# ViV99/slam-experiments

Measured on NVIDIA B200. Metric: hamming_pairs_per_sec, higher is better.
Workload: dtype u8

## Files before the change

### slam_experiments_b200/csrc/hm_tc.cu

```cuda
#include <math.h>
#include <stdlib.h>

#include <mutex>
#include <type_traits>

#include <cuda_fp16.h>

#include "hm_common.cuh"
#include "hm_tcgen05.cuh"

#ifndef HM_F4_TILE_N
#define HM_F4_TILE_N 128
#endif

namespace hm {

namespace {

constexpr int kRowBlock = 128;
constexpr int kMBlocks = 2;
constexpr int kBlockM = kRowBlock * kMBlocks;
constexpr int kSlabBytes = kRowBlock * 128;
constexpr int kPadRows = HM_PREPARED_TILE_ROWS;
constexpr int kTmemCols = 512;
// ... 59 lines not shown
    {
        const __half2 h = *reinterpret_cast<const __half2*>(&p);
        return hi ? __high2float(h) : __low2float(h);
    }
    static constexpr uint32_t kLowestBits = 0xFF800000u;
};

template <class C> __host__ __device__ constexpr int row_block_bytes() { return kRowBlock * C::kRowBytes; }
template <class C> __host__ __device__ constexpr int a_bytes() { return kMBlocks * row_block_bytes<C>(); }
template <class C> __host__ __device__ constexpr int b_stage_bytes() { return C::kTileN * C::kRowBytes; }
template <class C> __host__ __device__ constexpr int epilogue_warps() { return 4 * kMBlocks * C::kColSplit; }
template <class C> __host__ __device__ constexpr int control_warps() { return C::kRegisterHandover ? 4 : 2; }
template <class C> __host__ __device__ constexpr int threads() { return 32 * (control_warps<C>() + epilogue_warps<C>()); }
constexpr int kHandoverBytes = kBlockM * 16;
constexpr int kBarrierBytes = 512;
template <class C> __host__ __device__ constexpr int smem_bytes() { return 1024 + a_bytes<C>() + C::kStages * b_stage_bytes<C>() + kBarrierBytes + kHandoverBytes; }
static_assert((2 * CoreF4::kStages + 1 + 2 * CoreF4::kUnits) * 8 + 16 <= kBarrierBytes, "barrier block");
static_assert((2 * CoreI8::kStages + 1 + 2 * CoreI8::kUnits) * 8 + 16 <= kBarrierBytes, "barrier block");
__host__ __device__ constexpr int ct_gcd(int a, int b) { return b == 0 ? a : ct_gcd(b, a % b); }
template <class C> __host__ __device__ constexpr int issuer_period() { return C::kStages / ct_gcd(C::kStages, C::kUnits) * C::kUnits; }
constexpr int kScaleCols = 32;
constexpr int kScaleCol = kTmemCols - kScaleCols;
static_assert(CoreF4::kUnits * CoreF4::kTileN <= kScaleCol, "accumulator units must end before the scale factors");

struct PrepareParams {
    const uint8_t* bits;
    long long n, stride, batch_stride;
    long long padded_rows;
    uint8_t* out;
};

// ... 246 lines not shown
#define HM_SCAN_FLAT64 1
#endif
#ifndef HM_FLOOR_DENSE_TILES
#define HM_FLOOR_DENSE_TILES 32
#endif
#ifndef HM_FLOOR_LATE_MASK
#define HM_FLOOR_LATE_MASK 15
#endif

#ifndef HM_F4_A_TMEM
#define HM_F4_A_TMEM 0
#endif
constexpr int kATmemCol = 384;
constexpr int kATmemColsPerBlock = 32;

template <class C>
__device__ __forceinline__ void issue_half(int h, uint32_t a_block, uint32_t b_stage, uint32_t tmem_d, uint32_t idesc,
                                           uint32_t tmem_sf)
{
    constexpr int kHalf = C::kSlabs * 2;
#pragma unroll
    for (int jj = 0; jj < kHalf; ++jj) {
        const int j = h * kHalf + jj;
        const int slab = j >> 2, k = j & 3;
        const uint64_t db = ptx::kmajor_sw128_desc_from_lo(b_stage + ((slab * kSlabBytes + k * 32) >> 4));
        if constexpr (C::kScales && HM_F4_A_TMEM) {
            ptx::mma_mxf4_ts(tmem_d, a_block + 8 * j, db, idesc, tmem_sf, tmem_sf + kScaleCols / 2, j != 0);
        } else {
            const uint64_t da = ptx::kmajor_sw128_desc_from_lo(a_block + ((slab * kSlabBytes + k * 32) >> 4));
            if constexpr (C::kScales) ptx::mma_mxf4_ss(tmem_d, da, db, idesc, tmem_sf, tmem_sf + kScaleCols / 2, j != 0);
            else                      ptx::mma_i8_ss(tmem_d, da, db, idesc, j != 0);
        }
    }
}

template <class C, int kMode>
__device__ __forceinline__ void tc_knn2_body(const TcParams& P)
{
    constexpr bool kFloor = kMode == 1;
    using Acc = typename C::Acc;
    constexpr int kStages = C::kStages;
    constexpr int kUnits = C::kUnits;
    constexpr int kABytes = a_bytes<C>();
    constexpr int kBStageBytes = b_stage_bytes<C>();
    constexpr int kRowBlockBytes = row_block_bytes<C>();
    constexpr int kTileN = C::kTileN;

    extern __shared__ uint8_t smem_raw[];
    uint8_t* smem = smem_raw + ((1024u - (ptx::smem_u32(smem_raw) & 1023u)) & 1023u);
    uint8_t* smem_a = smem;
    uint8_t* smem_b = smem + kABytes;
    uint64_t* bars = reinterpret_cast<uint64_t*>(smem + kABytes + kStages * kBStageBytes);
    uint64_t* full_bar = bars;
    uint64_t* empty_bar = bars + kStages;
    uint64_t* a_full_bar = bars + 2 * kStages;
    uint64_t* tmem_full_bar = bars + 2 * kStages + 1;
    uint64_t* tmem_empty_bar = tmem_full_bar + kUnits;
    uint32_t* tmem_base_slot = reinterpret_cast<uint32_t*>(tmem_empty_bar + kUnits);
    uint32_t* smem_base_slot = tmem_base_slot + 2;
    ulonglong2* handover = reinterpret_cast<ulonglong2*>(smem + kABytes + kStages * kBStageBytes + kBarrierBytes);

    const int warp = __shfl_sync(0xffffffffu, threadIdx.x >> 5, 0);
    const int lane = threadIdx.x & 31;
    if (threadIdx.x == 0) cta_mark(P, 0);
    if (threadIdx.x == 0 && (blockIdx.x | blockIdx.y | blockIdx.z) == 0 && P.clock_probe) {
        unsigned long long t;
        asm volatile("mov.u64 %0, %%globaltimer;" : "=l"(t));
        P.clock_probe[0] = (long long)t;
        P.clock_probe[1] = clock64();
    }
    const int qb = blockIdx.x;
    const int split = blockIdx.y;
    const int b = blockIdx.z;

    const uint32_t cs = ptx::cluster_nctarank();
    const uint32_t crank = ptx::cluster_ctarank();
    const uint16_t cmask = (uint16_t)((1u << cs) - 1);
    const bool has_a = qb < P.q_blocks_valid;
    auto rows_present = [&]() -> long long { return P.nq_dyn ? min((long long)__ldg(P.nq_dyn + b), P.nq) : P.nq; };
    if (P.nq_dyn && (long long)(qb - (int)crank) * kBlockM >= rows_present()) return;

    const int tile_begin = split * P.tiles_per_split;
    const int tile_end = min(tile_begin + P.tiles_per_split, P.ntiles);
    const int my_tiles = tile_end - tile_begin;

    constexpr int kProducerWarp = kIssuerLast ? epilogue_warps<C>() : 0;
    constexpr int kIssuerWarp = kIssuerLast ? epilogue_warps<C>() + 1 : 1;
    constexpr int kFirstEpiWarp = kIssuerLast ? 0 : 2;
    static_assert(kIssuerLast || !C::kRegisterHandover, "the control warps must form the last warpgroup");
    static_assert(!C::kRegisterHandover || (epilogue_warps<C>() == 16 && threads<C>() == 640),
                  "the register budget (4 x 32 + 16 x 112 = 20 x 96) assumes 20 warps launched at 96 registers");
    if (warp == kProducerWarp && lane == 0) {
        *smem_base_slot = ptx::smem_u32(smem);
        for (int i = 0; i < kStages; ++i) {
            ptx::mbar_init(&full_bar[i], 1);
            ptx::mbar_init(&empty_bar[i], cs);
        }
        ptx::mbar_init(a_full_bar, 1);
        for (int i = 0; i < kUnits; ++i) {
            ptx::mbar_init(&tmem_full_bar[i], 1);
            ptx::mbar_init(&tmem_empty_bar[i], 4 * C::kColSplit);
        }
        ptx::fence_barrier_init();
        ptx::fence_proxy_async();
    } else if (warp == kIssuerWarp) {
        ptx::tmem_alloc(tmem_base_slot, kTmemCols);
        ptx::tmem_relinquish();
    }
    ptx::tc_fence_before();
    if (cs > 1) ptx::cluster_sync();
    else __syncthreads();
    ptx::tc_fence_after();
    const uint32_t tmem_base = *tmem_base_slot;

    if constexpr (C::kScales) {
        if (warp >= kFirstEpiWarp && warp < kFirstEpiWarp + 4) {
            uint32_t ones[32];
#pragma unroll
            for (int i = 0; i < 32; ++i) ones[i] = 0x7F7F7F7Fu;
            const uint32_t taddr = tmem_base + ((uint32_t)((warp & 3) * 32) << 16) + kScaleCol;
            static_assert(kScaleCols == 32, "one x32 store per lane quarter");
            ptx::tmem_st_32x32(taddr, ones);
// ... 42 lines not shown
                const int blk = o >> 10, rem = o & 1023;
                const int rr = (rem >> 3) & 7;
                const int r = ((rem >> 6) << 3) | rr;
                const int c = (rem & 7) ^ rr;
                const long long qrow = (long long)qb * kBlockM + blk * kRowBlock + r;
                uint4 v = make_uint4(0, 0, 0, 0);
                if (qrow < nq_eff) {
                    const long long srow = qidx ? (long long)__ldg(qidx + qrow) : qrow;
                    v = expand_bits_e2m1(*reinterpret_cast<const unsigned*>(qsrc + srow * P.q_bits_stride + c * 4));
                }
                reinterpret_cast<uint4*>(smem_a)[o] = v;
            }
            ptx::fence_proxy_async();
        }
        ptx::tc_fence_before();
        __syncthreads();
        ptx::tc_fence_after();
    }

    if (threadIdx.x == 0) cta_mark(P, 1);
    ulonglong2 my_keys = make_ulonglong2(kNoMatch, kNoMatch);
    long long my_row = -1;
    int my_row_in_cta = 0;

    auto run_producer = [&]() {
        if (lane == 0) {
            if (has_a && !P.qbits && !(C::kScales && HM_F4_A_TMEM)) {
                const uint8_t* qsrc = P.qprep + ((long long)b * P.q_padded + (long long)qb * kBlockM) * C::kRowBytes;
                ptx::mbar_arrive_expect_tx(a_full_bar, kABytes);
                ptx::bulk_g2s(smem_a, qsrc, kABytes, a_full_bar);
            }
            const uint8_t* tsrc = P.tprep + (long long)b * P.t_padded * C::kRowBytes;
            const uint32_t piece = kBStageBytes / cs;
            for (int i = 0; i < (HM_TC_EXPERIMENT >= 5 ? 0 : my_tiles); ++i) {
                const int stage = i % kStages;
                const uint32_t use = i / kStages;
#if HM_TC_EXPERIMENT < 4
                bounded_wait(&empty_bar[stage], (use & 1) ^ 1, P.error_flag);
#endif
                trace_mark(P, i, 0);
                ptx::mbar_arrive_expect_tx(&full_bar[stage], kBStageBytes);
                uint8_t* dst = smem_b + stage * kBStageBytes + crank * piece;
                const uint8_t* src = tsrc + (long long)(tile_begin + i) * kBStageBytes + crank * piece;
                if (cs > 1) ptx::bulk_g2s_multicast(dst, src, piece, &full_bar[stage], cmask);
                else        ptx::bulk_g2s(dst, src, piece, &full_bar[stage]);
            }
        }
    };
    auto run_issuer = [&]() {
        const bool leader = ptx::elect_one();
        const uint32_t idesc = C::kScales ? ptx::make_mxf4_idesc(kRowBlock, kTileN) : ptx::make_i8_idesc(kRowBlock, kTileN);
        constexpr bool kATmem = C::kScales && HM_F4_A_TMEM;
        const uint32_t a_addr = kATmem ? tmem_base + kATmemCol : ptx::smem_u32(smem_a) >> 4;
        constexpr uint32_t kABlockStep = kATmem ? (uint32_t)kATmemColsPerBlock : (uint32_t)(kRowBlockBytes >> 4);
        const uint32_t b_addr = ptx::smem_u32(smem_b) >> 4;
        const uint32_t tmem_sf = tmem_base + kScaleCol;
        if (has_a && !P.qbits && !(C::kScales && HM_F4_A_TMEM)) bounded_wait(a_full_bar, 0, P.error_flag);
        constexpr int kPeriod = issuer_period<C>();
        static_assert(kPeriod % kStages == 0 && (2 * kPeriod) % kUnits == 0 && ((2 * kPeriod / kUnits) & 1) == 0,
                      "unit parities must repeat with the period");
        uint32_t sphase = 0;
        bool ready0 = false;
        for (int base = 0; base < my_tiles; base += kPeriod) {
#pragma unroll
            for (int j = 0; j < kPeriod; ++j) {
                if (base + j < my_tiles) {
                    const int stage = j % kStages;
                    const uint32_t full_par = sphase ^ ((j / kStages) & 1);
                    const int unit_a = (2 * j) % kUnits, unit_b = (2 * j + 1) % kUnits;
                    const uint32_t par_a = (((2 * j) / kUnits) & 1) ^ 1, par_b = (((2 * j + 1) / kUnits) & 1) ^ 1;
                    const uint32_t b_stage = b_addr + stage * (kBStageBytes >> 4);
                    if (leader) trace_mark(P, base + j, 7);
                    if (!ready0) {
#if HM_TC_EXPERIMENT < 4
                        bounded_wait(&full_bar[stage], full_par, P.error_flag);
#endif
#if HM_TC_EXPERIMENT < 3
                        bounded_wait(&tmem_empty_bar[unit_a], par_a, P.error_flag);
#endif
                    }
                    if (leader) trace_mark(P, base + j, 1);
                    ptx::tc_fence_after();
                    if (leader) issue_half<C>(0, a_addr, b_stage, tmem_base + unit_a * kTileN, idesc, tmem_sf);
#if HM_TC_EXPERIMENT >= 3
                    const bool ready1 = true;
#else
                    const bool ready1 = __all_sync(0xffffffffu, ptx::mbar_test_wait(&tmem_empty_bar[unit_b], par_b));
#endif
                    if (leader) {
                        issue_half<C>(1, a_addr, b_stage, tmem_base + unit_a * kTileN, idesc, tmem_sf);
#if HM_TC_EXPERIMENT != 6 && HM_COMMIT_MODE == 0
                        ptx::tc_commit(&tmem_full_bar[unit_a]);
#endif
                    }
                    if (!ready1) bounded_wait(&tmem_empty_bar[unit_b], par_b, P.error_flag);
                    if (leader) trace_mark(P, base + j, 6);
                    ptx::tc_fence_after();
                    if (leader) issue_half<C>(0, a_addr + kABlockStep, b_stage, tmem_base + unit_b * kTileN, idesc, tmem_sf);
                    ready0 = false;
                    if (base + j + 1 < my_tiles) {
                        const int n = j + 1;
#if HM_TC_EXPERIMENT >= 4
                        ready0 = true;
#else
                        ready0 = __all_sync(0xffffffffu,
                                            ptx::mbar_test_wait(&full_bar[n % kStages], sphase ^ ((n / kStages) & 1))
#if HM_TC_EXPERIMENT < 3
                                            && ptx::mbar_test_wait(&tmem_empty_bar[(2 * n) % kUnits], (((2 * n) / kUnits) & 1) ^ 1)
#endif
                                            );
#endif
                    }
                    if (leader) {
                        issue_half<C>(1, a_addr + kABlockStep, b_stage, tmem_base + unit_b * kTileN, idesc, tmem_sf);
#if HM_TC_EXPERIMENT == 6 || HM_COMMIT_MODE == 1
                        ptx::tc_commit(&tmem_full_bar[unit_a]);
#endif
                        ptx::tc_commit(&tmem_full_bar[unit_b]);
                        if (cs > 1) ptx::tc_commit_multicast(&empty_bar[stage], cmask);
                        else        ptx::tc_commit(&empty_bar[stage]);
                    }
                }
            }
            sphase ^= (kPeriod / kStages) & 1;
        }
        __syncwarp();
    };
    auto run_epilogue = [&]() {
        constexpr int kCols = kTileN / C::kColSplit;
        const int quarter = warp & 3;
        const int mblk = ((warp - kFirstEpiWarp) >> 2) & 1;
        const int half = (warp - kFirstEpiWarp) >> 3;
        const int row_in_cta = mblk * kRowBlock + quarter * 32 + lane;
        const long long row = (long long)qb * kBlockM + row_in_cta;
        Top2<Acc> s;
        s.v1 = s.v2 = C::lowest();
        s.i1 = s.i2 = 0;
#pragma unroll
        for (int e = 0; e < 4; ++e) s.sa[e] = s.sb[e] = 0;
        s.f = C::floor_from(0);
#if HM_TC_TRACE
        s.slow = 0;
#endif
        unsigned floor_code = 0;
        const long long first_row = (long long)tile_begin * kTileN;
        const unsigned limit = (unsigned)min((long long)my_tiles * kTileN, P.nt - first_row);
        const uint32_t bars_addr = ptx::lds_volatile_u32(ptx::smem_u32(smem_base_slot)) + kABytes + kStages * kBStageBytes;
        const uint32_t unit_full_addr = bars_addr + (2 * kStages + 1) * 8;
        const uint32_t unit_empty_addr = unit_full_addr + kUnits * 8;
        int unit = mblk;
        uint32_t unit_use = 0;
        unsigned floor_pending = 0;
        auto refresh_floor = [&](int i) {
            if constexpr (kFloor) {
                if (i < HM_FLOOR_DENSE_TILES || (i & HM_FLOOR_LATE_MASK) == 0) {
                    floor_code = max(floor_code, floor_pending);
                    s.f = C::max2(s.f, C::floor_from(floor_code));
                    if (row < P.nq) {
                        unsigned* floor_ptr = P.row_floor + ((long long)b * P.nq + row);
                        const unsigned e = C::valid(s.v2) ? C::encode(s.v2) : 0u;
                        if (e > floor_code) { atomicMax(floor_ptr, e); floor_code = e; }
                        floor_pending = __ldcg(floor_ptr);
                    }
                }
// ... 28 lines not shown
                }
                scan_chunk<C, kMode>(r0, colbase, s);
                scan_chunk<C, kMode>(r1, colbase + 32, s);
                scan_chunk<C, kMode>(r2, colbase + 64, s);
                scan_chunk<C, kMode>(r3, colbase + 96, s);
            } else {
                if constexpr (kCols == 64) {
                    uint32_t r[64];
#if HM_TC_EXPERIMENT < 2
                    ptx::tmem_ld_32x64(taddr, r);
                    refresh_floor(i);
                    tmem_ld_fence64(r);
#endif
                    ptx::tc_fence_before();
                    __syncwarp();
                    if (HM_ARRIVE_ELECT ? ptx::elect_one() : lane == 0) ptx::mbar_arrive_addr(unit_empty_addr + unit * 8);
#if HM_TC_EXPERIMENT != 0
                    unit += 2;
                    if (unit >= kUnits) { unit -= kUnits; ++unit_use; }
                    return;
#endif
                    mask_tail<C, 64>(r, colbase, limit);
#if HM_SCAN_FLAT64
                    scan_chunk<C, kMode, 8>(r, colbase, s);
#else
                    scan_chunk<C, kMode>(r, colbase, s);
                    scan_chunk<C, kMode>(r + 32, colbase + 32, s);
#endif
                } else if constexpr (kCols == 32) {
                    uint32_t r[32];
                    ptx::tmem_ld_32x32(taddr, r);
// ... 49 lines not shown
        if (kMode != 2) fold_group(s.v2, s.i2, s.sb);
        else my_keys.y = kNoMatch;
        if (half == 1) handover[row_in_cta] = my_keys;
        else my_row = row;
        my_row_in_cta = row_in_cta;
    };

    auto run_tail = [&](auto worker_tag) {
        constexpr bool kWorker = decltype(worker_tag)::value;
        ptx::tc_fence_before();
        if (cs > 1) ptx::cluster_sync();
        else __syncthreads();
        if (kWorker && threadIdx.x == 0) cta_mark(P, 3);
        if (warp == kIssuerWarp) {
            ptx::tc_fence_after();
            ptx::tmem_dealloc(tmem_base, kTmemCols);
        }
        if (kWorker && my_row >= 0 && my_row < rows_present()) {
            if constexpr (C::kColSplit == 2) {
                const ulonglong2 o = handover[my_row_in_cta];
                top2_insert(my_keys.x, my_keys.y, o.x);
                top2_insert(my_keys.x, my_keys.y, o.y);
            }
            unsigned long long* out = P.out + (long long)split * P.out_split_stride + ((long long)b * P.nq + my_row) * 2;
            *reinterpret_cast<ulonglong2*>(out) = my_keys;
            if (!P.counters) select_candidate(P.sel, b, my_keys);
        }
        if (P.counters) {
            int* flag = reinterpret_cast<int*>(tmem_base_slot + 1);
            if (last_cta_arrives(&P.counters[(long long)b * gridDim.x + qb], (unsigned)P.splits, flag)) {
                const long long row = (long long)qb * kBlockM + threadIdx.x;
// ... 8 lines not shown
            }
        }
        if (kWorker && threadIdx.x == 0) cta_mark(P, 4);
        if (kWorker && threadIdx.x == 0 && (blockIdx.x | blockIdx.y | blockIdx.z) == 0 && P.clock_probe) {
            unsigned long long t;
            asm volatile("mov.u64 %0, %%globaltimer;" : "=l"(t));
            P.clock_probe[2] = (long long)t;
            P.clock_probe[3] = clock64();
        }
    };

    if constexpr (C::kRegisterHandover) {
        if (warp >= kProducerWarp) {
            asm volatile("setmaxnreg.dec.sync.aligned.u32 32;\n");
            if (warp == kProducerWarp) run_producer();
            else if (warp == kIssuerWarp) run_issuer();
            run_tail(std::false_type{});
            return;
        }
        asm volatile("setmaxnreg.inc.sync.aligned.u32 112;\n");
        run_epilogue();
        run_tail(std::true_type{});
    } else {
        if (warp == kProducerWarp) run_producer();
        else if (warp == kIssuerWarp) run_issuer();
        else run_epilogue();
        run_tail(std::true_type{});
    }
}

__global__ void __launch_bounds__(threads<CoreI8>(), 1) hm_i8_knn2_kernel(const TcParams P) { tc_knn2_body<CoreI8, 0>(P); }
__global__ void __launch_bounds__(threads<CoreF4>(), 1) hm_f4_knn2_kernel(const TcParams P) { tc_knn2_body<CoreF4, 0>(P); }
__global__ void __launch_bounds__(threads<CoreI8>(), 1) hm_i8_knn2_floor_kernel(const TcParams P) { tc_knn2_body<CoreI8, 1>(P); }
__global__ void __launch_bounds__(threads<CoreF4>(), 1) hm_f4_knn2_floor_kernel(const TcParams P) { tc_knn2_body<CoreF4, 1>(P); }
__global__ void __launch_bounds__(threads<CoreI8>(), 1) hm_i8_knn1_kernel(const TcParams P) { tc_knn2_body<CoreI8, 2>(P); }
__global__ void __launch_bounds__(threads<CoreF4>(), 1) hm_f4_knn1_kernel(const TcParams P) { tc_knn2_body<CoreF4, 2>(P); }

using KernelFn = void (*)(const TcParams);
template <class C> KernelFn kernel_of(int mode = 0);
template <> KernelFn kernel_of<CoreI8>(int mode) { return mode == 1 ? hm_i8_knn2_floor_kernel : mode == 2 ? hm_i8_knn1_kernel : hm_i8_knn2_kernel; }
template <> KernelFn kernel_of<CoreF4>(int mode) { return mode == 1 ? hm_f4_knn2_floor_kernel : mode == 2 ? hm_f4_knn1_kernel : hm_f4_knn2_kernel; }

struct TcPlan {
    int ntiles, splits, tiles_per_split;
    int cluster;
    long long qblocks;
};

int floor_max_tiles()
{
    static int v = -1;
    if (v < 0) {
        const char* e = getenv("HM_FLOOR_MAX_TILES");
        v = e ? atoi(e) : 0x7fffffff;
    }
    return v;
}

int floor_min_tiles_unsplit()
{
    static int v = -1;
    if (v < 0) {
        const char* e = getenv("HM_FLOOR_MIN_TILES_UNSPLIT");
// ... 18 lines not shown

int current_device_slot()
{
    int dev = 0;
    if (cudaGetDevice(&dev) != cudaSuccess) { cudaGetLastError(); dev = 0; }
    return (dev >= 0 && dev < kMaxDevices) ? dev : -1;
}

template <class C>
cudaError_t ensure_smem_opt_in()
{
    static bool done[kMaxDevices] = {};
    const int dev = current_device_slot();
    std::lock_guard<std::mutex> lock(g_launch_state_mu);
    if (dev >= 0 && done[dev]) return cudaSuccess;
    for (int mode = 0; mode < 3; ++mode) {
        const cudaError_t e = cudaFuncSetAttribute(kernel_of<C>(mode), cudaFuncAttributeMaxDynamicSharedMemorySize, smem_bytes<C>());
        if (e != cudaSuccess) return e;
    }
    if (dev >= 0) done[dev] = true;
    return cudaSuccess;
}

template <class C>
int resident_ctas(int cs, int sm_count)
{
    static int cache[kMaxDevices][5] = {};
    if (cs <= 1) return sm_count;
    const int dev = current_device_slot();
    if (dev >= 0) {
        std::lock_guard<std::mutex> lock(g_launch_state_mu);
        if (cache[dev][cs]) return cache[dev][cs];
    }
    int v = sm_count;
// ... 21 lines not shown
    }
    return v;
}

template <class C>
int prologue_tiles()
{
    static int v = -1;
    if (v < 0) {
        const char* e = getenv("HM_PROLOGUE_TILES");
        v = e ? atoi(e) : C::kPrologueTiles;
    }
    return v;
}

int cluster_min_tiles()
{
    static int v = -1;
    if (v < 0) {
        const char* e = getenv("HM_CLUSTER_MIN_TILES");
        v = e ? atoi(e) : 1024;
    }
    return v;
}

template <class C>
TcPlan plan_tc_cluster(long long nq, long long nt, int batch, int sm_count, int cluster)
{
    TcPlan pl{};
    const long long qb = ceil_div(nq, kBlockM);
// ... 41 lines not shown
    const TcPlan pl = plan_tc<C>(nq, nt, batch, sm_count);
    return (size_t)pl.splits * batch * nq * 2 * sizeof(unsigned long long);
}

inline size_t zeroed_bytes(long long row_blocks, long long rows) { return counters_bytes(row_blocks) + counters_bytes((rows + 1) / 2 * 2); }

template <class C>
size_t workspace_bytes_of(long long nq, long long nt, int batch, int sm_count, bool with_prepare)
{
    size_t b = 256 + zeroed_bytes(plan_tc<C>(nq, nt, batch, sm_count).qblocks * batch, nq * batch) + partials_bytes<C>(nq, nt, batch, sm_count);
    b = (b + 1023) & ~(size_t)1023;
    if (with_prepare) b += (size_t)(padded_rows<C>(nq) + padded_rows<C>(nt)) * C::kRowBytes * batch;
    return b;
}

template <class C>
int launch_prepared(const void* qprep, long long nq, const void* tprep, long long nt, int batch,
                    unsigned long long train_base, unsigned long long* out, void* ws, size_t ws_bytes,
                    int sm_count, cudaStream_t stream, const unsigned long long** out_partials,
                    int* out_groups, const ExchangeArgs* exchange, bool top1 = false, const QueryBits* qbits = nullptr,
                    const SelectArgs* select = nullptr)
{
    HM_CUDA_CHECK(ensure_smem_opt_in<C>());
    const TcPlan pl = plan_tc<C>(nq, nt, batch, sm_count);
    if ((long long)pl.ntiles * C::kTileN > (1ll << 32)) {
        set_error("train set too large for 32-bit trainIdx");
        return HM_ERR_UNSUPPORTED;
    }
    const bool keep_partials = out == nullptr;
    const size_t cbytes = zeroed_bytes(pl.qblocks * batch, nq * batch);
// ... 44 lines not shown
        P.out = partials;
        P.out_split_stride = rows * 2;
    }
    const bool fused_exchange = exchange && exchange->world > 1;
    if (fused_exchange) {
        if (batch != 1 || keep_partials) {
            set_error("fused exchange needs batch == 1 and an output buffer");
            return HM_ERR_INVALID_ARGUMENT;
        }
        static_assert(kBlockM == kExchangeRows, "flag granularity = query block");
        P.xch = *exchange;
        P.out = partials;
        P.out_split_stride = rows * 2;
    }
    bool zero_block = false;
    const bool floor_eligible = !top1 && !P.nq_dyn && pl.tiles_per_split <= floor_max_tiles() &&
                                (pl.splits > 1 || (C::kColSplit > 1 && pl.ntiles >= floor_min_tiles_unsplit()));
    if (floor_eligible) {
        P.row_floor = reinterpret_cast<unsigned*>(reinterpret_cast<uint8_t*>(counters) + counters_bytes(pl.qblocks * batch));
        zero_block = true;
    }
    if ((pl.splits > 1 || fused_exchange) && !keep_partials) {
        P.counters = counters;
        P.final_out = out;
        zero_block = true;
    } else if (!(pl.splits > 1 || keep_partials)) {
        P.out = out;
        P.out_split_stride = 0;
    }
    static const bool keep_floors = getenv("HM_KEEP_FLOORS") != nullptr;
    if (zero_block) HM_CUDA_CHECK(cudaMemsetAsync(counters, 0, keep_floors ? counters_bytes(pl.qblocks * batch) : cbytes, stream));
    if (pl.qblocks > 0x7FFFFFFFll || pl.splits > 65535 || batch > 65535) {
        set_error("grid too large");
        return HM_ERR_UNSUPPORTED;
    }
    cudaLaunchConfig_t cfg{};
    cfg.gridDim = dim3((unsigned)pl.qblocks, (unsigned)pl.splits, (unsigned)batch);
    cfg.blockDim = dim3(threads<C>());
    cfg.dynamicSmemBytes = smem_bytes<C>();
    cfg.stream = stream;
    cudaLaunchAttribute attr[1];
    attr[0].id = cudaLaunchAttributeClusterDimension;
    attr[0].val.clusterDim.x = (unsigned)pl.cluster;
    attr[0].val.clusterDim.y = 1;
    attr[0].val.clusterDim.z = 1;
    cfg.attrs = attr;
    cfg.numAttrs = 1;
    profile_mark(true, stream);
    cudaError_t le = cudaLaunchKernelEx(&cfg, kernel_of<C>(P.row_floor ? 1 : top1 ? 2 : 0), P);
    profile_mark(false, stream);
    if (le != cudaSuccess) {
        set_error("cudaLaunchKernelEx(tensor-core k-NN kernel, cluster %d) failed: %s", pl.cluster, cudaGetErrorString(le));
        return HM_ERR_CUDA;
    }
    HM_CUDA_CHECK(cudaGetLastError());
    if (trace_path) {
        static long long host[kTraceTiles * kTraceSlots];
        HM_CUDA_CHECK(cudaStreamSynchronize(stream));
        HM_CUDA_CHECK(cudaMemcpy(host, P.trace, sizeof(host), cudaMemcpyDeviceToHost));
        {
            const size_t nctas = (size_t)pl.qblocks * pl.splits * batch;
            long long* rec = (long long*)malloc(nctas * kCtaSlots * sizeof(long long));
            if (rec && cudaMemcpy(rec, P.trace + kTraceTiles * kTraceSlots, nctas * kCtaSlots * sizeof(long long), cudaMemcpyDeviceToHost) == cudaSuccess) {
                char path[1024];
// ... 153 lines not shown
    const size_t head = workspace_bytes_of<C>(p.nq, p.nt, p.batch, sm_count, false);
    uint8_t* tprep = static_cast<uint8_t*>(ws) + head + (size_t)padded_rows<C>(p.nq) * C::kRowBytes * p.batch;
    int rc = launch_prepare_of<C>(p.t, p.nt, p.t_stride, p.t_batch_stride, p.batch, tprep, stream);
    if (rc != HM_OK) return rc;
    QueryBits qb{};
    qb.bits = p.q; qb.stride = p.q_stride; qb.batch_stride = p.q_batch_stride;
    qb.index = list; qb.index_batch_stride = p.nq; qb.nq_dyn = count;
    return launch_prepared<C>(nullptr, p.nq, tprep, p.nt, p.batch, 0, out, ws, head, sm_count, stream, nullptr, nullptr,
                              nullptr, true, &qb);
}

template <class C>
static void describe_of(long long nq, long long nt, int batch, int sm_count, bool top1, char* buf, size_t n)
{
    const TcPlan pl = plan_tc<C>(nq, nt, batch, sm_count);
    const bool floor = !top1 && pl.splits > 1 && pl.tiles_per_split <= floor_max_tiles();
    snprintf(buf, n, "hm_%s_knn%s%s_kernel grid=(%lld,%d,%d) cluster=%d tiles_per_cta=%d", C::kScales ? "f4" : "i8",
             top1 ? "1" : "2", floor ? "_floor" : "", pl.qblocks, pl.splits, batch, pl.cluster, pl.tiles_per_split);
}

void describe_tc_launch(long long nq, long long nt, int batch, int sm_count, int variant, bool top1, char* buf, size_t n)
{
    if (variant == HM_VARIANT_F4) describe_of<CoreF4>(nq, nt, batch, sm_count, top1, buf, n);
    else                          describe_of<CoreI8>(nq, nt, batch, sm_count, top1, buf, n);
}

int launch_tc_knn2(const KnnProblem& p, unsigned long long* out, void* ws, size_t ws_bytes, int sm_count, int variant,
                   cudaStream_t stream)
{
    return variant == HM_VARIANT_F4 ? launch_knn2_of<CoreF4>(p, out, ws, ws_bytes, sm_count, stream)
                                    : launch_knn2_of<CoreI8>(p, out, ws, ws_bytes, sm_count, stream);
}

// ... 2 lines not shown
```

### slam_experiments_b200/csrc/hm_tcgen05.cuh

```cuda
#pragma once

#include <stdint.h>

namespace hm {
namespace ptx {

#ifndef HM_TRYWAIT_HINT_NS
#define HM_TRYWAIT_HINT_NS 0
#endif
#define HM_STR2(x) #x
#define HM_STR(x) HM_STR2(x)

__device__ __forceinline__ uint32_t smem_u32(const void* p)
{
    return static_cast<uint32_t>(__cvta_generic_to_shared(p));
}

__device__ __forceinline__ bool elect_one()
{
    uint32_t pred = 0;
    asm volatile(
        "{\n\t"
        ".reg .pred P;\n\t"
        "elect.sync _|P, 0xFFFFFFFF;\n\t"
// ... 109 lines not shown
        : "memory");
}

__device__ __forceinline__ uint32_t cluster_ctarank()
{
    uint32_t r;
    asm volatile("mov.u32 %0, %%cluster_ctarank;\n" : "=r"(r));
    return r;
}
__device__ __forceinline__ uint32_t cluster_nctarank()
{
    uint32_t r;
    asm volatile("mov.u32 %0, %%cluster_nctarank;\n" : "=r"(r));
    return r;
}
__device__ __forceinline__ void cluster_sync()
{
    asm volatile("barrier.cluster.arrive.release.aligned;\n" ::: "memory");
    asm volatile("barrier.cluster.wait.acquire.aligned;\n" ::: "memory");
}

__device__ __forceinline__ void tmem_alloc(uint32_t* smem_dst, uint32_t cols)
{
    asm volatile("tcgen05.alloc.cta_group::1.sync.aligned.shared::cta.b32 [%0], %1;\n" ::"r"(smem_u32(smem_dst)),
                 "r"(cols)
                 : "memory");
}
__device__ __forceinline__ void tmem_relinquish()
{
    asm volatile("tcgen05.relinquish_alloc_permit.cta_group::1.sync.aligned;\n" ::);
}
__device__ __forceinline__ void tmem_dealloc(uint32_t taddr, uint32_t cols)
{
    asm volatile("tcgen05.dealloc.cta_group::1.sync.aligned.b32 %0, %1;\n" ::"r"(taddr), "r"(cols));
}
__device__ __forceinline__ void tc_fence_before() { asm volatile("tcgen05.fence::before_thread_sync;\n" ::: "memory"); }
__device__ __forceinline__ void tc_fence_after() { asm volatile("tcgen05.fence::after_thread_sync;\n" ::: "memory"); }
__device__ __forceinline__ void tmem_ld_wait() { asm volatile("tcgen05.wait::ld.sync.aligned;\n" ::: "memory"); }

__device__ __forceinline__ void tc_commit(uint64_t* bar)
{
    asm volatile("tcgen05.commit.cta_group::1.mbarrier::arrive::one.shared::cluster.b64 [%0];\n" ::"r"(smem_u32(bar))
                 : "memory");
}

__device__ __forceinline__ void tc_commit_multicast(uint64_t* bar, uint16_t cta_mask)
{
    asm volatile(
        "tcgen05.commit.cta_group::1.mbarrier::arrive::one.shared::cluster.multicast::cluster.b64 [%0], %1;\n" ::"r"(
            smem_u32(bar)),
        "h"(cta_mask)
        : "memory");
}

__device__ __forceinline__ void mma_i8_ss(uint32_t tmem_d, uint64_t desc_a, uint64_t desc_b, uint32_t idesc,
                                          uint32_t accumulate)
{
    asm volatile(
        "{\n\t"
        ".reg .pred p;\n\t"
        "setp.ne.b32 p, %4, 0;\n\t"
        "tcgen05.mma.cta_group::1.kind::i8 [%0], %1, %2, %3, p;\n\t"
        "}\n" ::"r"(tmem_d),
        "l"(desc_a), "l"(desc_b), "r"(idesc), "r"(accumulate)
        : "memory");
}

__device__ __forceinline__ void mma_mxf4_ss(uint32_t tmem_d, uint64_t desc_a, uint64_t desc_b, uint32_t idesc,
                                            uint32_t tmem_sfa, uint32_t tmem_sfb, uint32_t accumulate)
{
    asm volatile(
        "{\n\t"
        ".reg .pred p;\n\t"
        "setp.ne.b32 p, %4, 0;\n\t"
        "tcgen05.mma.cta_group::1.kind::mxf4.block_scale.block32 [%0], %1, %2, %3, [%5], [%6], p;\n\t"
        "}\n" ::"r"(tmem_d),
        "l"(desc_a), "l"(desc_b), "r"(idesc), "r"(accumulate), "r"(tmem_sfa), "r"(tmem_sfb)
        : "memory");
}

__device__ __forceinline__ void mma_mxf4_ts(uint32_t tmem_d, uint32_t tmem_a, uint64_t desc_b, uint32_t idesc,
                                            uint32_t tmem_sfa, uint32_t tmem_sfb, uint32_t accumulate)
{
    asm volatile(
        "{\n\t"
        ".reg .pred p;\n\t"
        "setp.ne.b32 p, %4, 0;\n\t"
        "tcgen05.mma.cta_group::1.kind::mxf4.block_scale.block32 [%0], [%1], %2, %3, [%5], [%6], p;\n\t"
        "}\n" ::"r"(tmem_d),
        "r"(tmem_a), "l"(desc_b), "r"(idesc), "r"(accumulate), "r"(tmem_sfa), "r"(tmem_sfb)
// ... 81 lines not shown
```

Baseline: 13880.

## Use CTA-pair tcgen05 MMA for the mxf4 path in two-CTA clusters

Adds a cta_group::2 variant of the mxf4 k-NN kernel, used by default when the cluster size is 2. In it, one CTA issues 256-row MMAs covering both CTAs' query blocks, each CTA loads only half of every B tile, and the peer CTA's issuer warp becomes a relay that forwards barrier arrivals. The aim is to halve per-CTA B shared-memory traffic and stage size and to drop multicast, using paired tensor-core issue. The cost is more complex cross-CTA synchronisation, where mistakes in barrier counts or phases could hang the kernel or produce wrong results.

New measurement: 14620 (median of 6 runs). +5.4%, better.

```diff
diff --git a/slam_experiments_b200/csrc/hm_tc.cu b/slam_experiments_b200/csrc/hm_tc.cu
--- a/slam_experiments_b200/csrc/hm_tc.cu
+++ b/slam_experiments_b200/csrc/hm_tc.cu
@@ -97,7 +97,8 @@
 template <class C> __host__ __device__ constexpr int threads() { return 32 * (control_warps<C>() + epilogue_warps<C>()); }
 constexpr int kHandoverBytes = kBlockM * 16;
 constexpr int kBarrierBytes = 512;
-template <class C> __host__ __device__ constexpr int smem_bytes() { return 1024 + a_bytes<C>() + C::kStages * b_stage_bytes<C>() + kBarrierBytes + kHandoverBytes; }
+template <class C, bool k2Sm> __host__ __device__ constexpr int stage_bytes() { return b_stage_bytes<C>() / (k2Sm ? 2 : 1); }
+template <class C, bool k2Sm = false> __host__ __device__ constexpr int smem_bytes() { return 1024 + a_bytes<C>() + C::kStages * stage_bytes<C, k2Sm>() + kBarrierBytes + kHandoverBytes; }
 static_assert((2 * CoreF4::kStages + 1 + 2 * CoreF4::kUnits) * 8 + 16 <= kBarrierBytes, "barrier block");
 static_assert((2 * CoreI8::kStages + 1 + 2 * CoreI8::kUnits) * 8 + 16 <= kBarrierBytes, "barrier block");
 __host__ __device__ constexpr int ct_gcd(int a, int b) { return b == 0 ? a : ct_gcd(b, a % b); }
@@ -374,10 +375,11 @@
 constexpr int kATmemCol = 384;
 constexpr int kATmemColsPerBlock = 32;
 
-template <class C>
+template <class C, bool k2Sm = false>
 __device__ __forceinline__ void issue_half(int h, uint32_t a_block, uint32_t b_stage, uint32_t tmem_d, uint32_t idesc,
                                            uint32_t tmem_sf)
 {
+    static_assert(!k2Sm || (C::kScales && !HM_F4_A_TMEM), "the CTA-pair form exists for kind::mxf4 with A in shared memory");
     constexpr int kHalf = C::kSlabs * 2;
 #pragma unroll
     for (int jj = 0; jj < kHalf; ++jj) {
@@ -388,13 +390,14 @@
             ptx::mma_mxf4_ts(tmem_d, a_block + 8 * j, db, idesc, tmem_sf, tmem_sf + kScaleCols / 2, j != 0);
         } else {
             const uint64_t da = ptx::kmajor_sw128_desc_from_lo(a_block + ((slab * kSlabBytes + k * 32) >> 4));
-            if constexpr (C::kScales) ptx::mma_mxf4_ss(tmem_d, da, db, idesc, tmem_sf, tmem_sf + kScaleCols / 2, j != 0);
+            if constexpr (k2Sm) ptx::mma_mxf4_ss_2sm(tmem_d, da, db, idesc, tmem_sf, tmem_sf + kScaleCols / 2, j != 0);
+            else if constexpr (C::kScales) ptx::mma_mxf4_ss(tmem_d, da, db, idesc, tmem_sf, tmem_sf + kScaleCols / 2, j != 0);
             else                      ptx::mma_i8_ss(tmem_d, da, db, idesc, j != 0);
         }
     }
 }
 
-template <class C, int kMode>
+template <class C, int kMode, bool k2Sm = false>
 __device__ __forceinline__ void tc_knn2_body(const TcParams& P)
 {
     constexpr bool kFloor = kMode == 1;
@@ -403,6 +406,7 @@
     constexpr int kUnits = C::kUnits;
     constexpr int kABytes = a_bytes<C>();
     constexpr int kBStageBytes = b_stage_bytes<C>();
+    constexpr int kStageBytes = stage_bytes<C, k2Sm>();
     constexpr int kRowBlockBytes = row_block_bytes<C>();
     constexpr int kTileN = C::kTileN;
 
@@ -410,7 +414,7 @@
     uint8_t* smem = smem_raw + ((1024u - (ptx::smem_u32(smem_raw) & 1023u)) & 1023u);
     uint8_t* smem_a = smem;
     uint8_t* smem_b = smem + kABytes;
-    uint64_t* bars = reinterpret_cast<uint64_t*>(smem + kABytes + kStages * kBStageBytes);
+    uint64_t* bars = reinterpret_cast<uint64_t*>(smem + kABytes + kStages * kStageBytes);
     uint64_t* full_bar = bars;
     uint64_t* empty_bar = bars + kStages;
     uint64_t* a_full_bar = bars + 2 * kStages;
@@ -418,7 +422,7 @@
     uint64_t* tmem_empty_bar = tmem_full_bar + kUnits;
     uint32_t* tmem_base_slot = reinterpret_cast<uint32_t*>(tmem_empty_bar + kUnits);
     uint32_t* smem_base_slot = tmem_base_slot + 2;
-    ulonglong2* handover = reinterpret_cast<ulonglong2*>(smem + kABytes + kStages * kBStageBytes + kBarrierBytes);
+    ulonglong2* handover = reinterpret_cast<ulonglong2*>(smem + kABytes + kStages * kStageBytes + kBarrierBytes);
 
     const int warp = __shfl_sync(0xffffffffu, threadIdx.x >> 5, 0);
     const int lane = threadIdx.x & 31;
@@ -448,24 +452,27 @@
     constexpr int kIssuerWarp = kIssuerLast ? epilogue_warps<C>() + 1 : 1;
     constexpr int kFirstEpiWarp = kIssuerLast ? 0 : 2;
     static_assert(kIssuerLast || !C::kRegisterHandover, "the control warps must form the last warpgroup");
+    static_assert(!k2Sm || (C::kRegisterHandover && C::kTileN / C::kColSplit == 64 && HM_COMMIT_MODE == 0 && HM_TC_EXPERIMENT == 0),
+                  "the CTA-pair form is written for the kind::mxf4 shape (64-column items, handover, default commits)");
     static_assert(!C::kRegisterHandover || (epilogue_warps<C>() == 16 && threads<C>() == 640),
                   "the register budget (4 x 32 + 16 x 112 = 20 x 96) assumes 20 warps launched at 96 registers");
     if (warp == kProducerWarp && lane == 0) {
         *smem_base_slot = ptx::smem_u32(smem);
+        const uint32_t pair_arrivals = k2Sm && crank == 0 ? 2 : 1;
         for (int i = 0; i < kStages; ++i) {
-            ptx::mbar_init(&full_bar[i], 1);
-            ptx::mbar_init(&empty_bar[i], cs);
-        }
-        ptx::mbar_init(a_full_bar, 1);
+            ptx::mbar_init(&full_bar[i], pair_arrivals);
+            ptx::mbar_init(&empty_bar[i], k2Sm ? 1 : cs);
+        }
+        ptx::mbar_init(a_full_bar, pair_arrivals);
         for (int i = 0; i < kUnits; ++i) {
             ptx::mbar_init(&tmem_full_bar[i], 1);
-            ptx::mbar_init(&tmem_empty_bar[i], 4 * C::kColSplit);
+            ptx::mbar_init(&tmem_empty_bar[i], pair_arrivals * 4 * C::kColSplit);
         }
         ptx::fence_barrier_init();
         ptx::fence_proxy_async();
     } else if (warp == kIssuerWarp) {
-        ptx::tmem_alloc(tmem_base_slot, kTmemCols);
-        ptx::tmem_relinquish();
+        if constexpr (k2Sm) { ptx::tmem_alloc_2sm(tmem_base_slot, kTmemCols); ptx::tmem_relinquish_2sm(); }
+        else                { ptx::tmem_alloc(tmem_base_slot, kTmemCols); ptx::tmem_relinquish(); }
     }
     ptx::tc_fence_before();
     if (cs > 1) ptx::cluster_sync();
@@ -538,7 +545,8 @@
             ptx::fence_proxy_async();
         }
         ptx::tc_fence_before();
-        __syncthreads();
+        if (k2Sm) ptx::cluster_sync();
+        else __syncthreads();
         ptx::tc_fence_after();
     }
 
@@ -563,17 +571,18 @@
                 bounded_wait(&empty_bar[stage], (use & 1) ^ 1, P.error_flag);
 #endif
                 trace_mark(P, i, 0);
-                ptx::mbar_arrive_expect_tx(&full_bar[stage], kBStageBytes);
-                uint8_t* dst = smem_b + stage * kBStageBytes + crank * piece;
+                ptx::mbar_arrive_expect_tx(&full_bar[stage], k2Sm ? piece : kBStageBytes);
+                uint8_t* dst = smem_b + stage * kStageBytes + (k2Sm ? 0 : crank * piece);
                 const uint8_t* src = tsrc + (long long)(tile_begin + i) * kBStageBytes + crank * piece;
-                if (cs > 1) ptx::bulk_g2s_multicast(dst, src, piece, &full_bar[stage], cmask);
+                if (k2Sm) ptx::bulk_g2s(dst, src, piece, &full_bar[stage]);
+                else if (cs > 1) ptx::bulk_g2s_multicast(dst, src, piece, &full_bar[stage], cmask);
                 else        ptx::bulk_g2s(dst, src, piece, &full_bar[stage]);
             }
         }
     };
     auto run_issuer = [&]() {
         const bool leader = ptx::elect_one();
-        const uint32_t idesc = C::kScales ? ptx::make_mxf4_idesc(kRowBlock, kTileN) : ptx::make_i8_idesc(kRowBlock, kTileN);
+        const uint32_t idesc = C::kScales ? ptx::make_mxf4_idesc(k2Sm ? 2 * kRowBlock : kRowBlock, kTileN) : ptx::make_i8_idesc(kRowBlock, kTileN);
         constexpr bool kATmem = C::kScales && HM_F4_A_TMEM;
         const uint32_t a_addr = kATmem ? tmem_base + kATmemCol : ptx::smem_u32(smem_a) >> 4;
         constexpr uint32_t kABlockStep = kATmem ? (uint32_t)kATmemColsPerBlock : (uint32_t)(kRowBlockBytes >> 4);
@@ -593,7 +602,7 @@
                     const uint32_t full_par = sphase ^ ((j / kStages) & 1);
                     const int unit_a = (2 * j) % kUnits, unit_b = (2 * j + 1) % kUnits;
                     const uint32_t par_a = (((2 * j) / kUnits) & 1) ^ 1, par_b = (((2 * j + 1) / kUnits) & 1) ^ 1;
-                    const uint32_t b_stage = b_addr + stage * (kBStageBytes >> 4);
+                    const uint32_t b_stage = b_addr + stage * (kStageBytes >> 4);
                     if (leader) trace_mark(P, base + j, 7);
                     if (!ready0) {
 #if HM_TC_EXPERIMENT < 4
@@ -605,22 +614,23 @@
                     }
                     if (leader) trace_mark(P, base + j, 1);
                     ptx::tc_fence_after();
-                    if (leader) issue_half<C>(0, a_addr, b_stage, tmem_base + unit_a * kTileN, idesc, tmem_sf);
+                    if (leader) issue_half<C, k2Sm>(0, a_addr, b_stage, tmem_base + unit_a * kTileN, idesc, tmem_sf);
 #if HM_TC_EXPERIMENT >= 3
                     const bool ready1 = true;
 #else
                     const bool ready1 = __all_sync(0xffffffffu, ptx::mbar_test_wait(&tmem_empty_bar[unit_b], par_b));
 #endif
                     if (leader) {
-                        issue_half<C>(1, a_addr, b_stage, tmem_base + unit_a * kTileN, idesc, tmem_sf);
+                        issue_half<C, k2Sm>(1, a_addr, b_stage, tmem_base + unit_a * kTileN, idesc, tmem_sf);
 #if HM_TC_EXPERIMENT != 6 && HM_COMMIT_MODE == 0
-                        ptx::tc_commit(&tmem_full_bar[unit_a]);
+                        if (k2Sm) ptx::tc_commit_2sm_multicast(&tmem_full_bar[unit_a], 3);
+                        else ptx::tc_commit(&tmem_full_bar[unit_a]);
 #endif
                     }
                     if (!ready1) bounded_wait(&tmem_empty_bar[unit_b], par_b, P.error_flag);
                     if (leader) trace_mark(P, base + j, 6);
                     ptx::tc_fence_after();
-                    if (leader) issue_half<C>(0, a_addr + kABlockStep, b_stage, tmem_base + unit_b * kTileN, idesc, tmem_sf);
+                    if (leader) issue_half<C, k2Sm>(0, a_addr + kABlockStep, b_stage, tmem_base + unit_b * kTileN, idesc, tmem_sf);
                     ready0 = false;
                     if (base + j + 1 < my_tiles) {
                         const int n = j + 1;
@@ -636,17 +646,42 @@
 #endif
                     }
                     if (leader) {
-                        issue_half<C>(1, a_addr + kABlockStep, b_stage, tmem_base + unit_b * kTileN, idesc, tmem_sf);
+                        issue_half<C, k2Sm>(1, a_addr + kABlockStep, b_stage, tmem_base + unit_b * kTileN, idesc, tmem_sf);
 #if HM_TC_EXPERIMENT == 6 || HM_COMMIT_MODE == 1
                         ptx::tc_commit(&tmem_full_bar[unit_a]);
 #endif
-                        ptx::tc_commit(&tmem_full_bar[unit_b]);
-                        if (cs > 1) ptx::tc_commit_multicast(&empty_bar[stage], cmask);
-                        else        ptx::tc_commit(&empty_bar[stage]);
+                        if (k2Sm) {
+                            ptx::tc_commit_2sm_multicast(&tmem_full_bar[unit_b], 3);
+                            ptx::tc_commit_2sm_multicast(&empty_bar[stage], 3);
+                        } else {
+                            ptx::tc_commit(&tmem_full_bar[unit_b]);
+                            if (cs > 1) ptx::tc_commit_multicast(&empty_bar[stage], cmask);
+                            else        ptx::tc_commit(&empty_bar[stage]);
+                        }
                     }
                 }
             }
             sphase ^= (kPeriod / kStages) & 1;
+        }
+        __syncwarp();
+    };
+    auto run_relay = [&]() {
+        if (lane == 0) {
+            const uint32_t full0 = ptx::lds_volatile_u32(ptx::smem_u32(smem_base_slot)) + kABytes + kStages * kStageBytes;
+            const uint32_t a_full = full0 + 2 * kStages * 8;
+            const long long q_blk = blockIdx.x;
+            if (!P.qbits && q_blk - 1 < P.q_blocks_valid) {
+                if (q_blk < P.q_blocks_valid) bounded_wait_addr(a_full, 0, P.error_flag);
+                ptx::mbar_arrive_cluster(ptx::mapa_shared(a_full, 0));
+            }
+            const uint32_t peer_full = ptx::mapa_shared(full0, 0);
+            const int first = blockIdx.y * P.tiles_per_split;
+            const int n = min(first + P.tiles_per_split, P.ntiles) - first;
+            for (int i = 0; i < n; ++i) {
+                const int stage = i % kStages;
+                bounded_wait_addr(full0 + stage * 8, (uint32_t)(i / kStages) & 1, P.error_flag);
+                ptx::mbar_arrive_cluster(peer_full + stage * 8);
+            }
         }
         __syncwarp();
     };
@@ -669,9 +704,9 @@
         unsigned floor_code = 0;
         const long long first_row = (long long)tile_begin * kTileN;
         const unsigned limit = (unsigned)min((long long)my_tiles * kTileN, P.nt - first_row);
-        const uint32_t bars_addr = ptx::lds_volatile_u32(ptx::smem_u32(smem_base_slot)) + kABytes + kStages * kBStageBytes;
+        const uint32_t bars_addr = ptx::lds_volatile_u32(ptx::smem_u32(smem_base_slot)) + kABytes + kStages * kStageBytes;
         const uint32_t unit_full_addr = bars_addr + (2 * kStages + 1) * 8;
-        const uint32_t unit_empty_addr = unit_full_addr + kUnits * 8;
+        const uint32_t unit_empty_addr = k2Sm ? ptx::mapa_shared(unit_full_addr + kUnits * 8, 0) : unit_full_addr + kUnits * 8;
         int unit = mblk;
         uint32_t unit_use = 0;
         unsigned floor_pending = 0;
@@ -730,7 +765,10 @@
 #endif
                     ptx::tc_fence_before();
                     __syncwarp();
-                    if (HM_ARRIVE_ELECT ? ptx::elect_one() : lane == 0) ptx::mbar_arrive_addr(unit_empty_addr + unit * 8);
+                    if (HM_ARRIVE_ELECT ? ptx::elect_one() : lane == 0) {
+                        if (k2Sm) ptx::mbar_arrive_cluster(unit_empty_addr + unit * 8);
+                        else ptx::mbar_arrive_addr(unit_empty_addr + unit * 8);
+                    }
 #if HM_TC_EXPERIMENT != 0
                     unit += 2;
                     if (unit >= kUnits) { unit -= kUnits; ++unit_use; }
@@ -810,7 +848,8 @@
         if (kWorker && threadIdx.x == 0) cta_mark(P, 3);
         if (warp == kIssuerWarp) {
             ptx::tc_fence_after();
-            ptx::tmem_dealloc(tmem_base, kTmemCols);
+            if constexpr (k2Sm) ptx::tmem_dealloc_2sm(tmem_base, kTmemCols);
+            else ptx::tmem_dealloc(tmem_base, kTmemCols);
         }
         if (kWorker && my_row >= 0 && my_row < rows_present()) {
             if constexpr (C::kColSplit == 2) {
@@ -849,7 +888,10 @@
         if (warp >= kProducerWarp) {
             asm volatile("setmaxnreg.dec.sync.aligned.u32 32;\n");
             if (warp == kProducerWarp) run_producer();
-            else if (warp == kIssuerWarp) run_issuer();
+            else if (warp == kIssuerWarp) {
+                if (!k2Sm || ptx::cluster_ctarank() == 0) run_issuer();
+                else run_relay();
+            }
             run_tail(std::false_type{});
             return;
         }
@@ -865,16 +907,24 @@
 }
 
 __global__ void __launch_bounds__(threads<CoreI8>(), 1) hm_i8_knn2_kernel(const TcParams P) { tc_knn2_body<CoreI8, 0>(P); }
-__global__ void __launch_bounds__(threads<CoreF4>(), 1) hm_f4_knn2_kernel(const TcParams P) { tc_knn2_body<CoreF4, 0>(P); }
+template <bool k2Sm>
+__global__ void __launch_bounds__(threads<CoreF4>(), 1) hm_f4_knn2_kernel(const TcParams P) { tc_knn2_body<CoreF4, 0, k2Sm>(P); }
 __global__ void __launch_bounds__(threads<CoreI8>(), 1) hm_i8_knn2_floor_kernel(const TcParams P) { tc_knn2_body<CoreI8, 1>(P); }
-__global__ void __launch_bounds__(threads<CoreF4>(), 1) hm_f4_knn2_floor_kernel(const TcParams P) { tc_knn2_body<CoreF4, 1>(P); }
+template <bool k2Sm>
+__global__ void __launch_bounds__(threads<CoreF4>(), 1) hm_f4_knn2_floor_kernel(const TcParams P) { tc_knn2_body<CoreF4, 1, k2Sm>(P); }
 __global__ void __launch_bounds__(threads<CoreI8>(), 1) hm_i8_knn1_kernel(const TcParams P) { tc_knn2_body<CoreI8, 2>(P); }
-__global__ void __launch_bounds__(threads<CoreF4>(), 1) hm_f4_knn1_kernel(const TcParams P) { tc_knn2_body<CoreF4, 2>(P); }
+template <bool k2Sm>
+__global__ void __launch_bounds__(threads<CoreF4>(), 1) hm_f4_knn1_kernel(const TcParams P) { tc_knn2_body<CoreF4, 2, k2Sm>(P); }
 
 using KernelFn = void (*)(const TcParams);
-template <class C> KernelFn kernel_of(int mode = 0);
-template <> KernelFn kernel_of<CoreI8>(int mode) { return mode == 1 ? hm_i8_knn2_floor_kernel : mode == 2 ? hm_i8_knn1_kernel : hm_i8_knn2_kernel; }
-template <> KernelFn kernel_of<CoreF4>(int mode) { return mode == 1 ? hm_f4_knn2_floor_kernel : mode == 2 ? hm_f4_knn1_kernel : hm_f4_knn2_kernel; }
+template <class C> KernelFn kernel_of(int mode = 0, bool two_sm = false);
+template <> KernelFn kernel_of<CoreI8>(int mode, bool) { return mode == 1 ? hm_i8_knn2_floor_kernel : mode == 2 ? hm_i8_knn1_kernel : hm_i8_knn2_kernel; }
+template <> KernelFn kernel_of<CoreF4>(int mode, bool two_sm)
+{
+    if (two_sm) return mode == 1 ? hm_f4_knn2_floor_kernel<true> : mode == 2 ? hm_f4_knn1_kernel<true> : hm_f4_knn2_kernel<true>;
+    return mode == 1 ? hm_f4_knn2_floor_kernel<false> : mode == 2 ? hm_f4_knn1_kernel<false> : hm_f4_knn2_kernel<false>;
+}
+template <class C> int smem_bytes_of(bool two_sm) { return two_sm ? smem_bytes<C, true>() : smem_bytes<C, false>(); }
 
 struct TcPlan {
     int ntiles, splits, tiles_per_split;
@@ -882,6 +932,7 @@
     long long qblocks;
 };
 
+
 int floor_max_tiles()
 {
     static int v = -1;
@@ -930,10 +981,12 @@
     const int dev = current_device_slot();
     std::lock_guard<std::mutex> lock(g_launch_state_mu);
     if (dev >= 0 && done[dev]) return cudaSuccess;
-    for (int mode = 0; mode < 3; ++mode) {
-        const cudaError_t e = cudaFuncSetAttribute(kernel_of<C>(mode), cudaFuncAttributeMaxDynamicSharedMemorySize, smem_bytes<C>());
-        if (e != cudaSuccess) return e;
-    }
+    for (int mode = 0; mode < 3; ++mode)
+        for (int two_sm = 0; two_sm < (C::kScales ? 2 : 1); ++two_sm) {
+            const cudaError_t e = cudaFuncSetAttribute(kernel_of<C>(mode, two_sm), cudaFuncAttributeMaxDynamicSharedMemorySize,
+                                                       smem_bytes_of<C>(two_sm));
+            if (e != cudaSuccess) return e;
+        }
     if (dev >= 0) done[dev] = true;
     return cudaSuccess;
 }
@@ -985,6 +1038,16 @@
     return v;
 }
 
+bool f4_2sm_enabled()
+{
+    static int v = -1;
+    if (v < 0) {
+        const char* e = getenv("HM_F4_2SM");
+        v = e ? (atoi(e) != 0) : 1;
+    }
+    return v != 0;
+}
+
 int cluster_min_tiles()
 {
     static int v = -1;
@@ -1056,6 +1119,18 @@
     return b;
 }
 
+struct TcKernelChoice {
+    int mode;
+    bool two_sm;
+};
+template <class C>
+TcKernelChoice choose_kernel(const TcPlan& pl, bool top1, bool nq_dyn)
+{
+    const bool floor = !top1 && !nq_dyn && pl.tiles_per_split <= floor_max_tiles() &&
+                       (pl.splits > 1 || (C::kColSplit > 1 && pl.ntiles >= floor_min_tiles_unsplit()));
+    return {floor ? 1 : top1 ? 2 : 0, C::kScales && pl.cluster == 2 && f4_2sm_enabled()};
+}
+
 template <class C>
 int launch_prepared(const void* qprep, long long nq, const void* tprep, long long nt, int batch,
                     unsigned long long train_base, unsigned long long* out, void* ws, size_t ws_bytes,
@@ -1130,9 +1205,8 @@
         P.out_split_stride = rows * 2;
     }
     bool zero_block = false;
-    const bool floor_eligible = !top1 && !P.nq_dyn && pl.tiles_per_split <= floor_max_tiles() &&
-                                (pl.splits > 1 || (C::kColSplit > 1 && pl.ntiles >= floor_min_tiles_unsplit()));
-    if (floor_eligible) {
+    const TcKernelChoice kc = choose_kernel<C>(pl, top1, P.nq_dyn != nullptr);
+    if (kc.mode == 1) {
         P.row_floor = reinterpret_cast<unsigned*>(reinterpret_cast<uint8_t*>(counters) + counters_bytes(pl.qblocks * batch));
         zero_block = true;
     }
@@ -1153,7 +1227,7 @@
     cudaLaunchConfig_t cfg{};
     cfg.gridDim = dim3((unsigned)pl.qblocks, (unsigned)pl.splits, (unsigned)batch);
     cfg.blockDim = dim3(threads<C>());
-    cfg.dynamicSmemBytes = smem_bytes<C>();
+    cfg.dynamicSmemBytes = smem_bytes_of<C>(kc.two_sm);
     cfg.stream = stream;
     cudaLaunchAttribute attr[1];
     attr[0].id = cudaLaunchAttributeClusterDimension;
@@ -1163,7 +1237,7 @@
     cfg.attrs = attr;
     cfg.numAttrs = 1;
     profile_mark(true, stream);
-    cudaError_t le = cudaLaunchKernelEx(&cfg, kernel_of<C>(P.row_floor ? 1 : top1 ? 2 : 0), P);
+    cudaError_t le = cudaLaunchKernelEx(&cfg, kernel_of<C>(kc.mode, kc.two_sm), P);
     profile_mark(false, stream);
     if (le != cudaSuccess) {
         set_error("cudaLaunchKernelEx(tensor-core k-NN kernel, cluster %d) failed: %s", pl.cluster, cudaGetErrorString(le));
@@ -1347,9 +1421,10 @@
 static void describe_of(long long nq, long long nt, int batch, int sm_count, bool top1, char* buf, size_t n)
 {
     const TcPlan pl = plan_tc<C>(nq, nt, batch, sm_count);
-    const bool floor = !top1 && pl.splits > 1 && pl.tiles_per_split <= floor_max_tiles();
-    snprintf(buf, n, "hm_%s_knn%s%s_kernel grid=(%lld,%d,%d) cluster=%d tiles_per_cta=%d", C::kScales ? "f4" : "i8",
-             top1 ? "1" : "2", floor ? "_floor" : "", pl.qblocks, pl.splits, batch, pl.cluster, pl.tiles_per_split);
+    const TcKernelChoice kc = choose_kernel<C>(pl, top1, false);
+    snprintf(buf, n, "hm_%s_knn%s%s_kernel grid=(%lld,%d,%d) cluster=%d%s tiles_per_cta=%d", C::kScales ? "f4" : "i8",
+             top1 ? "1" : "2", kc.mode == 1 ? "_floor" : "", pl.qblocks, pl.splits, batch, pl.cluster,
+             kc.two_sm ? " cta_group=2" : "", pl.tiles_per_split);
 }
 
 void describe_tc_launch(long long nq, long long nt, int batch, int sm_count, int variant, bool top1, char* buf, size_t n)
diff --git a/slam_experiments_b200/csrc/hm_tcgen05.cuh b/slam_experiments_b200/csrc/hm_tcgen05.cuh
--- a/slam_experiments_b200/csrc/hm_tcgen05.cuh
+++ b/slam_experiments_b200/csrc/hm_tcgen05.cuh
@@ -147,6 +147,16 @@
     asm volatile("mov.u32 %0, %%cluster_nctarank;\n" : "=r"(r));
     return r;
 }
+__device__ __forceinline__ uint32_t mapa_shared(uint32_t smem_addr, uint32_t rank)
+{
+    uint32_t r;
+    asm volatile("mapa.shared::cluster.u32 %0, %1, %2;\n" : "=r"(r) : "r"(smem_addr), "r"(rank));
+    return r;
+}
+__device__ __forceinline__ void mbar_arrive_cluster(uint32_t cluster_addr)
+{
+    asm volatile("mbarrier.arrive.shared::cluster.b64 _, [%0];\n" ::"r"(cluster_addr) : "memory");
+}
 __device__ __forceinline__ void cluster_sync()
 {
     asm volatile("barrier.cluster.arrive.release.aligned;\n" ::: "memory");
@@ -166,6 +176,20 @@
 __device__ __forceinline__ void tmem_dealloc(uint32_t taddr, uint32_t cols)
 {
     asm volatile("tcgen05.dealloc.cta_group::1.sync.aligned.b32 %0, %1;\n" ::"r"(taddr), "r"(cols));
+}
+__device__ __forceinline__ void tmem_alloc_2sm(uint32_t* smem_dst, uint32_t cols)
+{
+    asm volatile("tcgen05.alloc.cta_group::2.sync.aligned.shared::cta.b32 [%0], %1;\n" ::"r"(smem_u32(smem_dst)),
+                 "r"(cols)
+                 : "memory");
+}
+__device__ __forceinline__ void tmem_relinquish_2sm()
+{
+    asm volatile("tcgen05.relinquish_alloc_permit.cta_group::2.sync.aligned;\n" ::);
+}
+__device__ __forceinline__ void tmem_dealloc_2sm(uint32_t taddr, uint32_t cols)
+{
+    asm volatile("tcgen05.dealloc.cta_group::2.sync.aligned.b32 %0, %1;\n" ::"r"(taddr), "r"(cols));
 }
 __device__ __forceinline__ void tc_fence_before() { asm volatile("tcgen05.fence::before_thread_sync;\n" ::: "memory"); }
 __device__ __forceinline__ void tc_fence_after() { asm volatile("tcgen05.fence::after_thread_sync;\n" ::: "memory"); }
@@ -181,6 +205,15 @@
 {
     asm volatile(
         "tcgen05.commit.cta_group::1.mbarrier::arrive::one.shared::cluster.multicast::cluster.b64 [%0], %1;\n" ::"r"(
+            smem_u32(bar)),
+        "h"(cta_mask)
+        : "memory");
+}
+
+__device__ __forceinline__ void tc_commit_2sm_multicast(uint64_t* bar, uint16_t cta_mask)
+{
+    asm volatile(
+        "tcgen05.commit.cta_group::2.mbarrier::arrive::one.shared::cluster.multicast::cluster.b64 [%0], %1;\n" ::"r"(
             smem_u32(bar)),
         "h"(cta_mask)
         : "memory");
@@ -207,6 +240,19 @@
         ".reg .pred p;\n\t"
         "setp.ne.b32 p, %4, 0;\n\t"
         "tcgen05.mma.cta_group::1.kind::mxf4.block_scale.block32 [%0], %1, %2, %3, [%5], [%6], p;\n\t"
+        "}\n" ::"r"(tmem_d),
+        "l"(desc_a), "l"(desc_b), "r"(idesc), "r"(accumulate), "r"(tmem_sfa), "r"(tmem_sfb)
+        : "memory");
+}
+
+__device__ __forceinline__ void mma_mxf4_ss_2sm(uint32_t tmem_d, uint64_t desc_a, uint64_t desc_b, uint32_t idesc,
+                                                uint32_t tmem_sfa, uint32_t tmem_sfb, uint32_t accumulate)
+{
+    asm volatile(
+        "{\n\t"
+        ".reg .pred p;\n\t"
+        "setp.ne.b32 p, %4, 0;\n\t"
+        "tcgen05.mma.cta_group::2.kind::mxf4.block_scale.block32 [%0], %1, %2, %3, [%5], [%6], p;\n\t"
         "}\n" ::"r"(tmem_d),
         "l"(desc_a), "l"(desc_b), "r"(idesc), "r"(accumulate), "r"(tmem_sfa), "r"(tmem_sfb)
         : "memory");
```
